# WallaceRao/svc_inference_pipeline

Hardware: AMD Instinct MI355X
Metric: converted audio sec/sec (RTF^-1) end-to-end, 10 s clips (higher is better)
Workload: dtype fp16; 1 GPU; batch=32/GPU x 10 s synthetic clips, Whisper-medium + PLMS-100 DiffSVC (speedup 10) + BigVGAN, fp16 MFMA operands (BigVGAN fp16) / fp32 accumulate, weight-split Whisper attention linears (all blocks) + MLP linears (blocks 0-3) + split-fp16 stem / DiffSVC head; global_batch=32, seq_len_frames=937, parallelism=dp1 (per-utterance shards, RCCL gather)

## Files before the change

### svc_inference_pipeline_amd/csrc/gate_ws.hip

```cpp
#include <type_traits>

#include "common.h"
#include "kernels.h"

#pragma clang diagnostic ignored "-Winline-asm"

namespace svc {

constexpr int GW_C = 384;
constexpr int GW_N = 768;
constexpr int GW_K = 3 * GW_C;
constexpr int GW_KS = 36;
constexpr int GW_KA_DEF = 24;
constexpr int GW_HALO = 8;
constexpr int GW_GR = 32;
constexpr int GW_NG = 5;
constexpr int GW_RROWS = GW_NG * GW_GR;
constexpr int GW_STRIDE = 800;
constexpr int GW_GBYTES = GW_GR * GW_STRIDE;
constexpr int GW_GPIECES = GW_GBYTES / 1024;
constexpr int GW_PART = GW_NG * GW_GBYTES;
constexpr int GW_ZERO = GW_PART + 2 * 4 * 2048;
constexpr int GW_TVT = GW_ZERO + 768;
constexpr int GW_MAXB = 1024;
constexpr int GW_STL = GW_TVT + GW_MAXB * 4;
constexpr int GW_NSTAMP = 128;
constexpr int GW_LDS = GW_STL;
constexpr int GW_LDS_STAMPS = GW_STL + 4 * GW_NSTAMP * 8;
constexpr int GW_PARTS = 42;
constexpr int GW_GRID = 256;
constexpr int GW_NT = 512;
constexpr uint32_t GW_OOR = 0x80000000u;
constexpr uint32_t GW_CFG = 0x00020000u;
static_assert(GW_GBYTES % 1024 == 0 && GW_STRIDE % 16 == 0, "ring geometry");

struct GateWsArgs {
  const f16* X;
  const f16* W;
  const float* bias;
  const f16* cp;
  int ld_cp;
  f16* y;
  int ldy;
  int M, T;
  int dil;
  const int* tv;
  int tv_mul, B;
  float invT;
  unsigned long long* stamps;
};

typedef uint32_t u32x4 __attribute__((ext_vector_type(4)));
__device__ __forceinline__ u32x4 gw_desc(const void* base, int64_t bytes) {
  const uint64_t a = (uint64_t)(uintptr_t)base;
  return u32x4{(uint32_t)a, (uint32_t)(a >> 32) & 0xffffu, (uint32_t)(bytes > 0 ? bytes : 0), GW_CFG};
}
__device__ __forceinline__ void gw_dma(u32x4 d, uint32_t voff, unsigned char* lds) {
  const uint32_t m0 =
      __builtin_amdgcn_readfirstlane((uint32_t)(uintptr_t)(__attribute__((address_space(3))) unsigned char*)lds);
  asm volatile("s_mov_b32 m0, %0\n\ts_nop 0\n\tbuffer_load_dwordx4 %1, %2, 0 offen lds"
               ::"s"(m0), "v"(voff), "s"(d) : "memory", "m0");
}
template <int N>
__device__ __forceinline__ void gw_vmwait() {
  static_assert(N >= 0 && N < 64, "vmcnt");
  asm volatile("s_waitcnt vmcnt(%0)" ::"n"(N) : "memory");
}
__device__ __forceinline__ void gw_barrier() {
  __builtin_amdgcn_sched_barrier(0);
  asm volatile("s_waitcnt lgkmcnt(0)" ::: "memory");
  __builtin_amdgcn_s_barrier();
  __builtin_amdgcn_sched_barrier(0);
}

union GwH4 { uint2 u; f16 h[4]; };

template <int DBG>
__device__ __forceinline__ void gw_stamp(unsigned char* smw, int i) {
  if constexpr ((DBG & 8) != 0)
    if (threadIdx.x == 256 && i < GW_NSTAMP)
      reinterpret_cast<unsigned long long*>(smw + GW_STL)[3 * GW_NSTAMP + i] = __builtin_amdgcn_s_memtime();
}
template <int DBG>
__device__ __forceinline__ void gw_stamp_lds(unsigned char* smw, int kind, int i, int thread) {
  if constexpr ((DBG & 8) != 0)
    if (threadIdx.x == thread && i < GW_NSTAMP)
      reinterpret_cast<unsigned long long*>(smw + GW_STL)[(kind - 1) * GW_NSTAMP + i] = __builtin_amdgcn_s_memtime();
}
template <int DBG>
__device__ __forceinline__ void gw_stamp_flush(const GateWsArgs& a, const unsigned char* smw, int kind, int n) {
  if constexpr ((DBG & 8) != 0) {
    const unsigned long long* src =
        reinterpret_cast<const unsigned long long*>(smw + GW_STL) + (kind == 0 ? 3 : kind - 1) * GW_NSTAMP;
    for (int i = threadIdx.x & 63; i < n && i < GW_NSTAMP; i += 64)
      a.stamps[((size_t)blockIdx.x * 4 + kind) * GW_NSTAMP + i] = src[i];
  }
}

__device__ __forceinline__ size_t gw_frag_index(int c, int p, int ks, int g) {
  return (size_t)(((c * 4 + p) * GW_KS + ks) * 2 + g) * 512;
}

struct GwRow {
  int m, bb, t, tvb;
  __device__ __forceinline__ void init(const GateWsArgs& a, const int* tvt, int m0) {
    m = m0;
    bb = (int)((float)m * a.invT);
    t = m - bb * a.T;
    if (t < 0) {
      --bb;
      t += a.T;
    } else if (t >= a.T) {
      ++bb;
      t -= a.T;
    }
    tvb = tvt[min(bb, a.B - 1)];
  }
  __device__ __forceinline__ void next(const GateWsArgs& a, const int* tvt) {
    m += 16;
    t += 16;
    const bool wrap = t >= a.T;
    t = wrap ? t - a.T : t;
    bb += wrap ? 1 : 0;
    tvb = tvt[min(bb, a.B - 1)];
  }
  __device__ __forceinline__ void bases(const GateWsArgs& a, int j, int fr, int fk, int base[3]) const {
    const bool row_ok = m < a.M;
    const int r0 = (16 * j) % GW_RROWS + GW_HALO + fr;
#pragma unroll
    for (int tap = 0; tap < 3; ++tap) {
      const int tp = t + (tap - 1) * a.dil;
      const bool ok = row_ok && tp >= 0 && tp < tvb;
      int rr = r0 + (tap - 1) * a.dil;
      rr = rr >= GW_RROWS ? rr - GW_RROWS : rr;
      base[tap] = (ok ? rr * GW_STRIDE : GW_ZERO) + fk * 16;
    }
  }
};

constexpr int GW_SG_VALU = 0x002, GW_SG_MFMA = 0x008, GW_SG_DSR = 0x100;

template <bool BF, int DBG, int GW_KA = GW_KA_DEF>
__global__ __launch_bounds__(GW_NT, 1) void gate_ws_kernel(GateWsArgs a) {
  using O = Op16<BF>;
  constexpr int GW_KB = GW_KS - GW_KA;
  static_assert(GW_KA >= GW_KB && GW_KB >= 4, "K split: the weight arrays are sized for the first wave; the epilogue's 4 "
                                             "elements need 4 segments");
  extern __shared__ __align__(16) unsigned char smw[];
  const int tid = threadIdx.x, lane = tid & 63;
  const int wave = __builtin_amdgcn_readfirstlane(tid >> 6);
  const int pair = wave & 3, kh = wave >> 2;
  const int fr = lane & 15, fk = lane >> 4;

  const int b = blockIdx.x, x = b & 7, j = b >> 3;
  int type, part;
  if (j < 30) {
    type = j % 6;
    part = x * 5 + j / 6;
  } else {
    const int s = (j - 30) * 8 + x;
    if (s >= 12) return;
    type = s % 6;
    part = 40 + s / 6;
  }
  const int nblk = (a.M + 15) >> 4;
  const int blk0 = (int)((int64_t)part * nblk / GW_PARTS);
  const int nsub = (int)((int64_t)(part + 1) * nblk / GW_PARTS) - blk0;
  if (nsub <= 0) return;
  const int r_begin = blk0 * 16;
  const int r_end = min(a.M, r_begin + nsub * 16);

  const int q = 2 * type + (pair >> 1), h = pair & 1;
  const int ng = 64 * q + 16 * h, nf = ng + 32;
  const int ch = 32 * q + 16 * h + 4 * fk;

  {
    int* tvt = reinterpret_cast<int*>(smw + GW_TVT);
    for (int i = tid; i < a.B; i += GW_NT) tvt[i] = a.tv ? min(a.T, a.tv[i] * a.tv_mul) : a.T;
  }
  for (int i = tid; i < 768 / 16; i += GW_NT) *reinterpret_cast<uint4*>(smw + GW_ZERO + i * 16) = make_uint4(0, 0, 0, 0);
  __syncthreads();
  const int* tvt = reinterpret_cast<const int*>(smw + GW_TVT);
  unsigned char* const part_buf = smw + GW_PART + pair * 2048;

  half8 wg[GW_KA], wf[GW_KA];
  auto load_w = [&](int ks0, auto n_) __attribute__((always_inline)) {
    constexpr int N = decltype(n_)::value;
    const f16* wb = a.W + gw_frag_index(type, pair, ks0, 0) + lane * 8;
#pragma unroll
    for (int s = 0; s < N; ++s) {
      wg[s] = *reinterpret_cast<const half8*>(wb + (size_t)(2 * s) * 512);
      wf[s] = *reinterpret_cast<const half8*>(wb + (size_t)(2 * s + 1) * 512);
    }
  };
  auto kloop = [&](const int base[3], int s_off, auto n_, floatx4& ag, floatx4& af, auto&& hook)
                   __attribute__((always_inline)) {
    constexpr int N = decltype(n_)::value;
    half8 av[5];
    auto rd = [&](int s) __attribute__((always_inline)) {
      const int ks = s_off + s;
      return *reinterpret_cast<const half8*>(smw + base[ks / 12] + (ks % 12) * 64);
    };
#pragma unroll
    for (int s = 0; s < 4; ++s) av[s] = rd(s);
#pragma unroll
    for (int s = 0; s < N; ++s) {
      __builtin_amdgcn_sched_barrier(0);
      if (s + 4 < N) av[(s + 4) % 5] = rd(s + 4);
      if constexpr (!(DBG & 2)) {
        ag = O::mfma(wg[s], av[s % 5], ag);
        af = O::mfma(wf[s], av[s % 5], af);
      }
      hook(s);
    }
    __builtin_amdgcn_sched_barrier(0);
  };
  auto no_hook = [](int) __attribute__((always_inline)) {};

  if (kh == 0) {
    const u32x4 dx = gw_desc(a.X, (int64_t)a.M * GW_C * 2);
    constexpr int PV = (GW_GPIECES + 3) / 4;
    uint32_t pc[PV];
#pragma unroll
    for (int v = 0; v < PV; ++v) {
      const int u = (pair + 4 * v) * 64 + lane;
      const int r = u / 50, c = u - r * 50;
      pc[v] = c < 48 ? (uint32_t)(r * GW_C * 2 + c * 16) : GW_OOR;
    }
    const bool seven = pair + 4 * (PV - 1) < GW_GPIECES;
    auto issue = [&](int g) __attribute__((always_inline)) {
      const uint32_t base = (uint32_t)((r_begin - GW_HALO + g * GW_GR) * (GW_C * 2));
      unsigned char* dst = smw + (g % GW_NG) * GW_GBYTES + pair * 1024;
#pragma unroll
      for (int v = 0; v < PV; ++v)
        if (v < PV - 1 || seven) gw_dma(dx, base + pc[v], dst + v * 4096);
    };
    issue(0);
    issue(1);
    load_w(0, std::integral_constant<int, GW_KA>());
    __builtin_amdgcn_s_waitcnt(0x0f70);
    issue(2);
    issue(3);
    issue(4);
    GwRow row;
    row.init(a, tvt, r_begin + fr);
    gw_barrier();
    auto step = [&](int k) __attribute__((always_inline)) {
      if ((k & 1) && k >= 3) issue((k + 7) / 2);
      int base[3];
      row.bases(a, k, fr, fk, base);
      floatx4 ag = {0.f, 0.f, 0.f, 0.f}, af = {0.f, 0.f, 0.f, 0.f};
      kloop(base, 0, std::integral_constant<int, GW_KA>(), ag, af, no_hook);
      unsigned char* pb = part_buf + (k & 1) * 8192 + lane * 16;
      *reinterpret_cast<floatx4*>(pb) = ag;
      *reinterpret_cast<floatx4*>(pb + 1024) = af;
      row.next(a, tvt);
      gw_stamp_lds<DBG>(smw, 1, k, 0);
      if (k & 1) {
        if (seven) gw_vmwait<3 * PV>(); else gw_vmwait<3 * (PV - 1)>();
      } else {
        if (seven) gw_vmwait<2 * PV>(); else gw_vmwait<2 * (PV - 1)>();
      }
      gw_stamp_lds<DBG>(smw, 2, k, 0);
      gw_barrier();
    };
    for (int k = 0; k < nsub; ++k) step(k);
    gw_barrier();
    gw_vmwait<0>();
    if (wave == 0) {
      gw_stamp_flush<DBG>(a, smw, 1, nsub);
      gw_stamp_flush<DBG>(a, smw, 2, nsub);
    }
  } else {
    const __amdgpu_buffer_rsrc_t rcp =
        __builtin_amdgcn_make_buffer_rsrc(const_cast<f16*>(a.cp), (short)0, a.M * a.ld_cp * 2, GW_CFG);
    const __amdgpu_buffer_rsrc_t ry = __builtin_amdgcn_make_buffer_rsrc(a.y, (short)0, a.M * a.ldy * 2, GW_CFG);
    gw_stamp<DBG>(smw, 0);
    load_w(GW_KA, std::integral_constant<int, GW_KB>());
    const float4 bg = *reinterpret_cast<const float4*>(a.bias + ng + 4 * fk);
    const float4 bfv = *reinterpret_cast<const float4*>(a.bias + nf + 4 * fk);
    auto load_cp = [&](int blk, GwH4* dst) __attribute__((always_inline)) {
      const uint32_t vo = (uint32_t)(r_begin + blk * 16 + fr) * (uint32_t)(a.ld_cp * 2);
      dst[0].u = __builtin_bit_cast(uint2, __builtin_amdgcn_raw_buffer_load_b64(rcp, vo + (ng + 4 * fk) * 2, 0, 0));
      dst[1].u = __builtin_bit_cast(uint2, __builtin_amdgcn_raw_buffer_load_b64(rcp, vo + (nf + 4 * fk) * 2, 0, 0));
    };
    GwH4 c0[2], c1[2], c2[2];
    floatx4 pg = {0.f, 0.f, 0.f, 0.f}, pf = {0.f, 0.f, 0.f, 0.f};
    GwRow row;
    row.init(a, tvt, r_begin + fr);
    gw_stamp<DBG>(smw, 1);
    gw_barrier();
    __builtin_amdgcn_s_setprio(1);
    gw_stamp<DBG>(smw, 2);
    auto gate_el = [&](int i, const GwH4* cp, const floatx4& ag, const floatx4& af) __attribute__((always_inline)) {
      if constexpr ((DBG & 4) != 0) {
        return (f16)(ag[i] + af[(i + 1) & 3]);
      } else {
        const float b_g = i == 0 ? bg.x : (i == 1 ? bg.y : (i == 2 ? bg.z : bg.w));
        const float b_f = i == 0 ? bfv.x : (i == 1 ? bfv.y : (i == 2 ? bfv.z : bfv.w));
        return O::enc_lo(gate_act(ag[i] + b_g + O::dec(cp[0].h[i]), af[i] + b_f + O::dec(cp[1].h[i])));
      }
    };
    auto store_blk = [&](int blk, const GwH4& pk) __attribute__((always_inline)) {
      const int m = r_begin + blk * 16 + fr;
      const uint32_t vo = m < r_end ? (uint32_t)m * (uint32_t)(a.ldy * 2) + (uint32_t)ch * 2 : GW_OOR;
      buffer_store_b64(pk.u, ry, vo);
    };
    auto epilogue = [&](int blk, const GwH4* cp, const floatx4& ag, const floatx4& af) __attribute__((always_inline)) {
      GwH4 pk;
#pragma unroll
      for (int i = 0; i < 4; ++i) pk.h[i] = gate_el(i, cp, ag, af);
      store_blk(blk, pk);
    };
    auto mfma_blk = [&](int blk, floatx4& ag, floatx4& af, auto&& hook) __attribute__((always_inline)) {
      int base[3];
      row.bases(a, blk, fr, fk, base);
      const unsigned char* pb = part_buf + (blk & 1) * 8192 + lane * 16;
      ag = *reinterpret_cast<const floatx4*>(pb);
      af = *reinterpret_cast<const floatx4*>(pb + 1024);
      kloop(base, GW_KA, std::integral_constant<int, GW_KB>(), ag, af, hook);
      row.next(a, tvt);
    };
    auto end_step = [&](int k) __attribute__((always_inline)) {
      gw_stamp_lds<DBG>(smw, 3, k, 256);
      gw_barrier();
      gw_stamp<DBG>(smw, 3 + k);
    };
    auto steady = [&](int k, GwH4* ls, const GwH4* es) __attribute__((always_inline)) {
      load_cp(k, ls);
      floatx4 ag, af;
      const floatx4 eg = pg, ef = pf;
      GwH4 pk;
      auto hook = [&](int s) __attribute__((always_inline)) {
#pragma unroll
        for (int i = 0; i < 4; ++i)
          if (s == (i + 1) * GW_KB / 4 - 1) pk.h[i] = gate_el(i, es, eg, ef);
        if (s == GW_KB - 1) store_blk(k - 2, pk);
      };
      mfma_blk(k - 1, ag, af, hook);
      pg = ag;
      pf = af;
      end_step(k);
    };
    load_cp(0, c0);
    end_step(0);
    if (nsub >= 2) load_cp(1, c1);
    mfma_blk(0, pg, pf, no_hook);
    end_step(1);
    int k = 2;
    for (; k + 3 <= nsub; k += 3) {
      steady(k, c2, c0);
      steady(k + 1, c0, c1);
      steady(k + 2, c1, c2);
    }
    if (k < nsub) steady(k++, c2, c0);
    if (k < nsub) steady(k++, c0, c1);
    auto epi_set = [&](int blk) __attribute__((always_inline)) {
      switch (blk % 3) {
        case 0: epilogue(blk, c0, pg, pf); break;
        case 1: epilogue(blk, c1, pg, pf); break;
        default: epilogue(blk, c2, pg, pf); break;
      }
    };
    if (nsub >= 2) {
      floatx4 ag, af;
      mfma_blk(nsub - 1, ag, af, no_hook);
      epi_set(nsub - 2);
      pg = ag;
      pf = af;
      end_step(nsub);
    }
    epi_set(nsub - 1);
    if (wave == 4) {
      gw_stamp_flush<DBG>(a, smw, 3, nsub + 1);
      gw_stamp_flush<DBG>(a, smw, 0, nsub + 4);
    }
  }
}

__global__ void gate_ws_pack_kernel(const f16* __restrict__ W, f16* __restrict__ Wf) {
  const int i = blockIdx.x * blockDim.x + threadIdx.x;
  if (i >= GW_N * GW_K / 8) return;
  const int lane = i & 63;
  int r = i >> 6;
  const int g = r & 1;
  r >>= 1;
  const int ks = r % GW_KS;
  r /= GW_KS;
  const int p = r & 3, c = r >> 2;
  const int n = 64 * (2 * c + (p >> 1)) + 16 * (p & 1) + 32 * g + (lane & 15);
  const int k = 32 * ks + 8 * (lane >> 4);
  *reinterpret_cast<uint4*>(Wf + (size_t)i * 8) = *reinterpret_cast<const uint4*>(W + (size_t)n * GW_K + k);
}

int gate_ws_pack(const f16* W, int ldw, f16* Wf, hipStream_t s) {
  SVC_REQUIRE(ldw == GW_K && ((uintptr_t)W & 15) == 0 && ((uintptr_t)Wf & 15) == 0, "gate_ws_pack: ldw %d", ldw);
  hipLaunchKernelGGL(gate_ws_pack_kernel, dim3(cdiv(GW_N * GW_K / 8, 256)), dim3(256), 0, s, W, Wf);
  SVC_LAUNCH_CHECK();
  return SVC_OK;
}
size_t gate_ws_pack_elems() { return (size_t)GW_N * GW_K; }

unsigned long long* gate_ws_stamps = nullptr;
int gate_ws_nstamp() { return 4 * GW_NSTAMP; }

static bool gate_ws_fits_shape(const ConvGemmArgs& a, const EpiArgs& e) {
  const int d = a.tap_mul;
  return e.kind == EPI_GATE && e.cp && e.y16 && e.bias && a.Cp == GW_C && a.Cvalid == GW_C && a.ldx == GW_C &&
         a.K == GW_K && a.Kpad == GW_K && a.N == GW_N && (d == 1 || d == 2 || d == 4 || d == 8) && a.tap_add == -d &&
         a.istride == 1 && a.T_in == a.T_out && a.T_out >= 16 && a.B <= GW_MAXB && e.ld_cp % 4 == 0 && e.ldy16 % 4 == 0 &&
         (int64_t)a.B * a.T_out * std::max(e.ld_cp, std::max(e.ldy16, GW_C)) * 2 < (1ll << 30);
}

bool gate_ws_fits(const ConvGemmArgs& a, const EpiArgs& e) { return a.Wfrag && gate_ws_fits_shape(a, e); }

int gate_ws(const ConvGemmArgs& a, const EpiArgs& e, hipStream_t s) {
  SVC_REQUIRE(gate_ws_fits(a, e), "gate_ws: not the DiffSVC dilated-conv gate shape");
  SVC_REQUIRE(((uintptr_t)a.X & 15) == 0 && ((uintptr_t)a.Wfrag & 15) == 0 && ((uintptr_t)e.cp & 7) == 0 &&
                  ((uintptr_t)e.y16 & 7) == 0 && ((uintptr_t)e.bias & 15) == 0,
              "gate_ws: alignment");
  const int M = a.B * a.T_out;
  if (M == 0) return SVC_OK;
  static const int dbg = getenv("SVC_GWS_DBG") ? atoi(getenv("SVC_GWS_DBG")) : 0;
  GateWsArgs g{a.X, a.Wfrag, e.bias, e.cp, e.ld_cp, e.y16, e.ldy16, M, a.T_out, a.tap_mul, a.tv, a.tv_mul, a.B,
               1.0f / (float)a.T_out, gate_ws_stamps};
  static const int ka = getenv("SVC_GWS_KA") ? atoi(getenv("SVC_GWS_KA")) : GW_KA_DEF;
  const void* fn = a.bf16 ? (const void*)gate_ws_kernel<true, 0> : (const void*)gate_ws_kernel<false, 0>;
  if (!a.bf16 && gate_ws_stamps) fn = (const void*)gate_ws_kernel<false, 8>;
  else if (!a.bf16 && dbg == 2) fn = (const void*)gate_ws_kernel<false, 2>;
  else if (!a.bf16 && dbg == 4) fn = (const void*)gate_ws_kernel<false, 4>;
  else if (!a.bf16 && ka == 18) fn = (const void*)gate_ws_kernel<false, 0, 18>;
  else if (!a.bf16 && ka == 22) fn = (const void*)gate_ws_kernel<false, 0, 22>;
  const int lds = fn == (const void*)gate_ws_kernel<false, 8> ? GW_LDS_STAMPS : GW_LDS;
  if (int st = ensure_dyn_lds(fn, lds)) return st;
  const int tok = prof_begin("gate_ws<16x128>", 2.0 * M * (double)GW_N * GW_K, 0.0, s);
  void* args[] = {&g};
  SVC_HIP_CHECK(hipLaunchKernel(fn, dim3(GW_GRID), dim3(GW_NT), args, lds, s));
  prof_end(tok, s);
  SVC_LAUNCH_CHECK();
  return SVC_OK;
}



}
```

Baseline: 942.1 audio-s/s.

## Stage gate conditioning tiles into LDS via producer-wave DMA ring

```diff
diff --git a/svc_inference_pipeline_amd/csrc/gate_ws.hip b/svc_inference_pipeline_amd/csrc/gate_ws.hip
--- a/svc_inference_pipeline_amd/csrc/gate_ws.hip
+++ b/svc_inference_pipeline_amd/csrc/gate_ws.hip
@@ -19,14 +19,18 @@
 constexpr int GW_STRIDE = 800;
 constexpr int GW_GBYTES = GW_GR * GW_STRIDE;
 constexpr int GW_GPIECES = GW_GBYTES / 1024;
-constexpr int GW_PART = GW_NG * GW_GBYTES;
+constexpr int GW_CPR = GW_NG * GW_GBYTES;
+constexpr int GW_CPS = 3;
+constexpr int GW_CPSLOT = 16 * 256;
+constexpr int GW_PART = GW_CPR + GW_CPS * GW_CPSLOT;
 constexpr int GW_ZERO = GW_PART + 2 * 4 * 2048;
 constexpr int GW_TVT = GW_ZERO + 768;
 constexpr int GW_MAXB = 1024;
 constexpr int GW_STL = GW_TVT + GW_MAXB * 4;
-constexpr int GW_NSTAMP = 128;
+constexpr int GW_NSTAMP = 64;
 constexpr int GW_LDS = GW_STL;
 constexpr int GW_LDS_STAMPS = GW_STL + 4 * GW_NSTAMP * 8;
+static_assert(GW_LDS_STAMPS <= 160 * 1024 && GW_CPR % 1024 == 0, "LDS budget");
 constexpr int GW_PARTS = 42;
 constexpr int GW_GRID = 256;
 constexpr int GW_NT = 512;
@@ -219,6 +223,7 @@
 
   if (kh == 0) {
     const u32x4 dx = gw_desc(a.X, (int64_t)a.M * GW_C * 2);
+    const u32x4 dc = gw_desc(a.cp, (int64_t)a.M * a.ld_cp * 2);
     constexpr int PV = (GW_GPIECES + 3) / 4;
     uint32_t pc[PV];
 #pragma unroll
@@ -235,8 +240,17 @@
       for (int v = 0; v < PV; ++v)
         if (v < PV - 1 || seven) gw_dma(dx, base + pc[v], dst + v * 4096);
     };
+    const int cpr = 4 * pair + (lane >> 4);
+    const uint32_t pcc = (uint32_t)(cpr * a.ld_cp * 2 + type * 256 + (((lane & 15) ^ cpr) * 16));
+    int cps = 0;
+    auto issue_cp = [&](int j) __attribute__((always_inline)) {
+      gw_dma(dc, (uint32_t)(r_begin + 16 * j) * (uint32_t)(a.ld_cp * 2) + pcc, smw + GW_CPR + cps + pair * 1024);
+      cps = cps == (GW_CPS - 1) * GW_CPSLOT ? 0 : cps + GW_CPSLOT;
+    };
     issue(0);
     issue(1);
+    issue_cp(0);
+    issue_cp(1);
     load_w(0, std::integral_constant<int, GW_KA>());
     __builtin_amdgcn_s_waitcnt(0x0f70);
     issue(2);
@@ -246,6 +260,7 @@
     row.init(a, tvt, r_begin + fr);
     gw_barrier();
     auto step = [&](int k) __attribute__((always_inline)) {
+      if (k >= 2) issue_cp(k);
       if ((k & 1) && k >= 3) issue((k + 7) / 2);
       int base[3];
       row.bases(a, k, fr, fk, base);
@@ -256,15 +271,22 @@
       *reinterpret_cast<floatx4*>(pb + 1024) = af;
       row.next(a, tvt);
       gw_stamp_lds<DBG>(smw, 1, k, 0);
-      if (k & 1) {
+      if (k < 2) {
         if (seven) gw_vmwait<3 * PV>(); else gw_vmwait<3 * (PV - 1)>();
+      } else if (k == 2) {
+        if (seven) gw_vmwait<2 * PV + 1>(); else gw_vmwait<2 * (PV - 1) + 1>();
       } else {
-        if (seven) gw_vmwait<2 * PV>(); else gw_vmwait<2 * (PV - 1)>();
+        if (seven) gw_vmwait<PV + 1>(); else gw_vmwait<PV>();
       }
       gw_stamp_lds<DBG>(smw, 2, k, 0);
       gw_barrier();
     };
     for (int k = 0; k < nsub; ++k) step(k);
+    if (nsub >= 4 && !(nsub & 1)) {
+      if (seven) gw_vmwait<PV>(); else gw_vmwait<PV - 1>();
+    } else {
+      gw_vmwait<0>();
+    }
     gw_barrier();
     gw_vmwait<0>();
     if (wave == 0) {
@@ -272,19 +294,20 @@
       gw_stamp_flush<DBG>(a, smw, 2, nsub);
     }
   } else {
-    const __amdgpu_buffer_rsrc_t rcp =
-        __builtin_amdgcn_make_buffer_rsrc(const_cast<f16*>(a.cp), (short)0, a.M * a.ld_cp * 2, GW_CFG);
     const __amdgpu_buffer_rsrc_t ry = __builtin_amdgcn_make_buffer_rsrc(a.y, (short)0, a.M * a.ldy * 2, GW_CFG);
     gw_stamp<DBG>(smw, 0);
     load_w(GW_KA, std::integral_constant<int, GW_KB>());
     const float4 bg = *reinterpret_cast<const float4*>(a.bias + ng + 4 * fk);
     const float4 bfv = *reinterpret_cast<const float4*>(a.bias + nf + 4 * fk);
-    auto load_cp = [&](int blk, GwH4* dst) __attribute__((always_inline)) {
-      const uint32_t vo = (uint32_t)(r_begin + blk * 16 + fr) * (uint32_t)(a.ld_cp * 2);
-      dst[0].u = __builtin_bit_cast(uint2, __builtin_amdgcn_raw_buffer_load_b64(rcp, vo + (ng + 4 * fk) * 2, 0, 0));
-      dst[1].u = __builtin_bit_cast(uint2, __builtin_amdgcn_raw_buffer_load_b64(rcp, vo + (nf + 4 * fk) * 2, 0, 0));
-    };
-    GwH4 c0[2], c1[2], c2[2];
+    const int cg = 8 * (pair >> 1) + 2 * h + (fk >> 1);
+    const unsigned char* cp_g = smw + GW_CPR + fr * 256 + ((cg ^ fr) * 16) + (fk & 1) * 8;
+    const unsigned char* cp_f = smw + GW_CPR + fr * 256 + (((cg + 4) ^ fr) * 16) + (fk & 1) * 8;
+    int cps = 0;
+    auto read_cp = [&](GwH4* dst) __attribute__((always_inline)) {
+      dst[0].u = *reinterpret_cast<const uint2*>(cp_g + cps);
+      dst[1].u = *reinterpret_cast<const uint2*>(cp_f + cps);
+      cps = cps == (GW_CPS - 1) * GW_CPSLOT ? 0 : cps + GW_CPSLOT;
+    };
     floatx4 pg = {0.f, 0.f, 0.f, 0.f}, pf = {0.f, 0.f, 0.f, 0.f};
     GwRow row;
     row.init(a, tvt, r_begin + fr);
@@ -306,8 +329,9 @@
       const uint32_t vo = m < r_end ? (uint32_t)m * (uint32_t)(a.ldy * 2) + (uint32_t)ch * 2 : GW_OOR;
       buffer_store_b64(pk.u, ry, vo);
     };
-    auto epilogue = [&](int blk, const GwH4* cp, const floatx4& ag, const floatx4& af) __attribute__((always_inline)) {
-      GwH4 pk;
+    auto epilogue = [&](int blk, const floatx4& ag, const floatx4& af) __attribute__((always_inline)) {
+      GwH4 cp[2], pk;
+      read_cp(cp);
 #pragma unroll
       for (int i = 0; i < 4; ++i) pk.h[i] = gate_el(i, cp, ag, af);
       store_blk(blk, pk);
@@ -326,11 +350,11 @@
       gw_barrier();
       gw_stamp<DBG>(smw, 3 + k);
     };
-    auto steady = [&](int k, GwH4* ls, const GwH4* es) __attribute__((always_inline)) {
-      load_cp(k, ls);
+    auto steady = [&](int k) __attribute__((always_inline)) {
+      GwH4 es[2], pk;
+      read_cp(es);
       floatx4 ag, af;
       const floatx4 eg = pg, ef = pf;
-      GwH4 pk;
       auto hook = [&](int s) __attribute__((always_inline)) {
 #pragma unroll
         for (int i = 0; i < 4; ++i)
@@ -342,35 +366,19 @@
       pf = af;
       end_step(k);
     };
-    load_cp(0, c0);
     end_step(0);
-    if (nsub >= 2) load_cp(1, c1);
     mfma_blk(0, pg, pf, no_hook);
     end_step(1);
-    int k = 2;
-    for (; k + 3 <= nsub; k += 3) {
-      steady(k, c2, c0);
-      steady(k + 1, c0, c1);
-      steady(k + 2, c1, c2);
-    }
-    if (k < nsub) steady(k++, c2, c0);
-    if (k < nsub) steady(k++, c0, c1);
-    auto epi_set = [&](int blk) __attribute__((always_inline)) {
-      switch (blk % 3) {
-        case 0: epilogue(blk, c0, pg, pf); break;
-        case 1: epilogue(blk, c1, pg, pf); break;
-        default: epilogue(blk, c2, pg, pf); break;
-      }
-    };
+    for (int k = 2; k < nsub; ++k) steady(k);
     if (nsub >= 2) {
       floatx4 ag, af;
       mfma_blk(nsub - 1, ag, af, no_hook);
-      epi_set(nsub - 2);
+      epilogue(nsub - 2, pg, pf);
       pg = ag;
       pf = af;
       end_step(nsub);
     }
-    epi_set(nsub - 1);
+    epilogue(nsub - 1, pg, pf);
     if (wave == 4) {
       gw_stamp_flush<DBG>(a, smw, 3, nsub + 1);
       gw_stamp_flush<DBG>(a, smw, 0, nsub + 4);
@@ -408,7 +416,7 @@
   const int d = a.tap_mul;
   return e.kind == EPI_GATE && e.cp && e.y16 && e.bias && a.Cp == GW_C && a.Cvalid == GW_C && a.ldx == GW_C &&
          a.K == GW_K && a.Kpad == GW_K && a.N == GW_N && (d == 1 || d == 2 || d == 4 || d == 8) && a.tap_add == -d &&
-         a.istride == 1 && a.T_in == a.T_out && a.T_out >= 16 && a.B <= GW_MAXB && e.ld_cp % 4 == 0 && e.ldy16 % 4 == 0 &&
+         a.istride == 1 && a.T_in == a.T_out && a.T_out >= 16 && a.B <= GW_MAXB && e.ld_cp % 8 == 0 && e.ld_cp >= GW_N && e.ldy16 % 4 == 0 &&
          (int64_t)a.B * a.T_out * std::max(e.ld_cp, std::max(e.ldy16, GW_C)) * 2 < (1ll << 30);
 }
 
@@ -416,7 +424,7 @@
 
 int gate_ws(const ConvGemmArgs& a, const EpiArgs& e, hipStream_t s) {
   SVC_REQUIRE(gate_ws_fits(a, e), "gate_ws: not the DiffSVC dilated-conv gate shape");
-  SVC_REQUIRE(((uintptr_t)a.X & 15) == 0 && ((uintptr_t)a.Wfrag & 15) == 0 && ((uintptr_t)e.cp & 7) == 0 &&
+  SVC_REQUIRE(((uintptr_t)a.X & 15) == 0 && ((uintptr_t)a.Wfrag & 15) == 0 && ((uintptr_t)e.cp & 15) == 0 &&
                   ((uintptr_t)e.y16 & 7) == 0 && ((uintptr_t)e.bias & 15) == 0,
               "gate_ws: alignment");
   const int M = a.B * a.T_out;
```

New measurement: 944.4 audio-s/s (median of 6 runs). Within noise of the previous version (+0.2%).
